# FFTAI/Wiki-GRx-Gym

Hardware: AMD Instinct MI355X
Metric: env-steps/sec GR1T1 rough-terrain @4096 envs (higher is better)
Workload: dtype f32

## Files before the change

wiki-grx-gym_amd/csrc/grx_step_kernel_body.inc:

```
    static_assert(!DBG || W == 1 || W == 4 || W == 8, "the debug injection path exists for the one-wave layout and the pipelines");
    KP P = GRX_PARAMS(Pg);
    constexpr int NTHR = 64 * W;
    constexpr bool PIPE = W >= 4;
    __shared__ KTables s_tab;
    constexpr int OBS_BYTES = EPB * GRX_NUM_OBS * 4, PRI_BYTES = EPB * PRS * 4, RW_BYTES = PIPE ? REWIN_FLOATS * 64 * 4 : 0;
    constexpr int POST_BYTES = OBS_BYTES + PRI_BYTES + RW_BYTES, PHYS_BYTES = (W == 2 || W == 8 ? 2 : 1) * RC_BYTES;
    static_assert(OBS_BYTES % 16 == 0 && PRI_BYTES % 16 == 0 && RC_BYTES % 16 == 0, "arena pieces must stay 16-byte aligned");
    constexpr int FOOTFR_BYTES = RC_FR4 * 64 * 16, ANCH_BYTES = 16 * 64 * 4;
    constexpr int TAIL_BYTES = PIPE ? PHYS_BYTES + FOOTFR_BYTES + ANCH_BYTES : PHYS_BYTES;
#ifdef GRX_FAKE_ARENA
    __shared__ __attribute__((aligned(16))) char s_arena[GRX_FAKE_ARENA];
#else
    __shared__ __attribute__((aligned(16))) char s_arena[POST_BYTES > TAIL_BYTES ? POST_BYTES : TAIL_BYTES];
#endif
    float* const s_obs = reinterpret_cast<float*>(s_arena);
    float* const s_pri = reinterpret_cast<float*>(s_arena + OBS_BYTES);
    float* const s_rw = reinterpret_cast<float*>(s_arena + OBS_BYTES + PRI_BYTES);
    static_assert(!PIPE || PHYS_BYTES >= OBS_BYTES + PRI_BYTES, "foot frames + s_anch must sit behind the staging rows, in the arena's tail");
    float4* const s_footfr = reinterpret_cast<float4*>(s_arena + PHYS_BYTES);
    float* const s_anch = reinterpret_cast<float*>(s_arena + PHYS_BYTES + FOOTFR_BYTES);
    __shared__ float s_stat[NSTAT];
    __shared__ float s_base[W == 2 ? 13 * EPB : 1];
    __shared__ float4 s_bq[PIPE ? 4 * EPB : 1];
    __shared__ __attribute__((aligned(16))) float s_wr[W == 2 ? 32 * 64 : (PIPE ? 8 * 64 : 1)];
    __shared__ float4 s_q[PIPE ? Q4 * 64 : 1];
    __shared__ float4 s_wc[PIPE ? WC4 * 64 : 1];
    __shared__ float4 s_pb[PIPE ? (LEG * PB4 + 2) * 64 : 1];
    __shared__ uint32_t s_nz[PIPE ? NZB * 4 * 64 : 1];
    __shared__ float4 s_rr[PIPE ? 5 * 64 : 1];
    __shared__ __attribute__((aligned(16))) char s_self[PIPE ? SELF_BYTES : 16];
    __shared__ float s_rwp[PIPE ? 64 : 1];
    __shared__ float s_hp[PIPE ? 4 * EPB : 1];
    __shared__ float s_hsum[PIPE ? W * 64 : 1];
    __shared__ float s_bho[W == 8 && HF ? 4 * 64 : 1];
    __shared__ float s_tp[PIPE ? 2 * 64 : 1];
    __shared__ float4 s_xk[W == 8 ? 9 * 64 : 1];
    __shared__ float4 s_sb[W == 8 ? 5 * 64 : 1];
    __shared__ float4 s_fx[W == 8 && LPL == 2 ? 8 * 64 : 1];
    __shared__ int s_flag[FL_COUNT];
    const PipeLds L = {s_bq, s_q, s_wc, s_pb, reinterpret_cast<float4*>(s_wr), s_flag, s_xk, s_sb, s_fx};
    const int tid = threadIdx.x;
#ifdef GRX_PROFILE_SECTIONS
    if (tid == 0) { P.prof[(size_t)blockIdx.x * GRX_PROF_SLOTS + 136] = (long long)__builtin_amdgcn_s_memrealtime(); P.prof[(size_t)blockIdx.x * GRX_PROF_SLOTS + 137] = clock64(); }
#endif
#ifndef GRX_W8_ROLES
#define GRX_W8_ROLES 0x76543210u
#endif
    const int wv_hw = __builtin_amdgcn_readfirstlane(tid >> 6);
    const int wv = W == 8 ? (int)((GRX_W8_ROLES >> (4 * wv_hw)) & 7u) : wv_hw;
    const RareBuf RB = rare_carve(s_arena + (W == 2 && wv == 1 ? RC_BYTES : 0));
    {
        const uint32_t* src = reinterpret_cast<const uint32_t*>(P.tables);
        uint32_t* dst = reinterpret_cast<uint32_t*>(&s_tab);
        for (int i = tid; i < (int)(sizeof(KTables) / 4); i += NTHR) dst[i] = src[i];
        if (tid < NSTAT) s_stat[tid] = 0.f;
        if (tid < FL_COUNT) s_flag[tid] = 0;
    }
    __syncthreads();
    if (wv == (W == 8 ? 3 : W - 1)) stats_fold_previous(P, sq, tid & 63);
    const int N = P.N;
    const int lane = tid & 63, el = lane_env(lane), side = lane_side(lane), half = lane_half(lane);
    const int grp = step_group();
    const int e_raw = grp * EPB + el;
    const bool act = e_raw < N;
    const bool act0 = act && half == 0;
    int e = act ? e_raw : N - 1;
    const SideConst& C = s_tab.side[side];
    const uint32_t genv = (uint32_t)(P.env_offset + e);
    const uint32_t step = (uint32_t)common_step;
    const int nh = P.nh, npri = P.num_pri_obs;
    const float dtp = P.sim_dt * (float)P.decimation;
    const int j0 = side * LEG;

#ifndef GRX_W8_PRIO
#define GRX_W8_PRIO 0u
#endif
    if (W == 8 && GRX_W8_PRIO) {
        const int pr = (int)((GRX_W8_PRIO >> (4 * wv)) & 3u);
        if (pr == 1) __builtin_amdgcn_s_setprio(1);
        else if (pr == 2) __builtin_amdgcn_s_setprio(2);
        else if (pr == 3) __builtin_amdgcn_s_setprio(3);
    }
    if (W >= 2 && wv != 0) {
        const float mu = 0.5f * (P.terrain_friction + P.friction[e]);
        float hmax = 0.0f;
        if (HF) {
            const float x0 = P.root[0 * (size_t)N + e], y0 = P.root[1 * (size_t)N + e];
            int ci = min(max((int)((x0 + P.border_size) / (P.horizontal_scale * (float)GRX_COARSE)), 0), P.coarse_rows - 1);
            int cj = min(max((int)((y0 + P.border_size) / (P.horizontal_scale * (float)GRX_COARSE)), 0), P.coarse_cols - 1);
            hmax = P.coarse_max[(size_t)ci * P.coarse_cols + cj];
        }
        LaneState hs;
        hs.anchor_on = 0;
        LinkPrep w3_lp;
        V3 w3_rows[11];
        if (PIPE) {
#if defined(GRX_REG_CONSTS) && GRX_REG_CONSTS >= 2
            const SideConst Ch = C;
#define GRX_HELPER_C Ch
#else
#define GRX_HELPER_C C
#endif
#ifndef GRX_W8_REGC
#define GRX_W8_REGC 0x76
#endif
#define GRX_HC(w) ((W == 8 && !((GRX_W8_REGC >> (w)) & 1)) ? C : GRX_HELPER_C)
            const float bm = P.base_m[e];
            const V3 bc = v3(P.base_c[e], P.base_c[(size_t)N + e], P.base_c[2 * (size_t)N + e]);
            const S3 bI = {P.base_I[e], P.base_I[(size_t)N + e], P.base_I[2 * (size_t)N + e],
                           P.base_I[3 * (size_t)N + e], P.base_I[4 * (size_t)N + e], P.base_I[5 * (size_t)N + e]};
            if (wv == 1) {
                const bool want_noise = P.add_noise && !noise_in;
                const int noise_seq = P.decimation >= 2 ? P.decimation - 2 : 0;
                auto noise_out = [&](const int seq) {
                    if (want_noise && seq == noise_seq) {
                        U4 nzb[NZB];
                        noise_blocks(P, genv, step, side, nzb);
                        uint32_t* z = s_nz + lane;
#pragma unroll
                        for (int b = 0; b < NZB; ++b) { z[(b * 4 + 0) * 64] = nzb[b].x; z[(b * 4 + 1) * 64] = nzb[b].y; z[(b * 4 + 2) * 64] = nzb[b].z; z[(b * 4 + 3) * 64] = nzb[b].w; }
                    }
                };
                if (DBG) noise_out(noise_seq);
                else self_loop<HF, HF && W != 8, W == 8>(P, s_tab, GRX_HC(1), RB, s_footfr, self_carve(s_self), P.friction[e], L, lane, el, side, noise_out);
            } else if (wv == 2) {
                constexpr int NA = 4 / LPL;
#pragma unroll
                for (int i = 0; i < NA; ++i) {
                    const int gi = NA * half + i;
                    hs.ax[i] = P.anchors[(size_t)((side * 4 + gi) * 3 + 0) * N + e];
                    hs.ay[i] = P.anchors[(size_t)((side * 4 + gi) * 3 + 1) * N + e];
                    hs.vimp[i] = P.anchors[(size_t)((side * 4 + gi) * 3 + 2) * N + e];
                    if (hs.vimp[i] != 0.0f) hs.anchor_on |= (1u << i);
                }
                V3 rpy_acc = v3(0.f, 0.f, 0.f);
                if (!DBG) chain_contact_loop<HF, W == 8 ? 0 : (HF ? 2 : 5)>(P, GRX_HC(2), C, RB, s_footfr, mu, hmax, 1.0f - 0.5f * (P.terrain_restitution + P.restitution[e]), hs, L, lane, el, side, rpy_acc);
                float* a_ = s_anch + (lane - half);
                if (half == 0) { a_[13 * 64] = rpy_acc.x; a_[14 * 64] = rpy_acc.y; a_[15 * 64] = rpy_acc.z; }
#pragma unroll
                for (int i = 0; i < NA; ++i) { const int gi = NA * half + i; a_[gi * 64] = hs.ax[i]; a_[(4 + gi) * 64] = hs.ay[i]; a_[(9 + gi) * 64] = hs.vimp[i]; }
                {
                    const uint32_t mine = hs.anchor_on << (NA * half);
                    a_[8 * 64] = __uint_as_float(LPL == 1 ? mine : (mine | __float_as_uint(half_swap(__uint_as_float(mine)))));
                }
            } else if (wv == 3) {
                if (DBG) { s_tp[lane] = dbg[(size_t)DBG_TERM_CONTACT * N + e]; s_tp[64 + lane] = 0.f; }
                else base_contact_loop<HF, W == 8>(P, s_tab, GRX_HC(3), RB, mu, hmax, bm, bc, bI, L, lane, el, side, s_tp, w3_lp, w3_rows, s_footfr, P.friction[e]);
            } else if (DBG) {
            } else if (wv == 7) {
                RareBuf RB7 = rare_carve(s_arena + RC_BYTES);
                RB7.fchain = RB.fchain;
                chain_rare_loop<HF>(P, s_tab, GRX_HC(7), RB7, mu, hmax, L, lane, el, side);
            } else if (wv == 4) {
                chain_bias_loop<3, 4>(P, GRX_HC(4), C, L, lane, el);
            } else if (wv == 6) {
                if (LPL == 1) chain_bias_loop<0, 2, true>(P, GRX_HC(6), C, L, lane, el, &s_tab, &RB, s_footfr, side, P.friction[e]);
                else chain_bias_loop<0, 2>(P, GRX_HC(6), C, L, lane, el);
            } else if (wv == 5) {
                base_service_loop(P, GRX_HC(5), C, bm, bc, bI, L, lane, el);
            }
            float es_w1[NT], es_w3[NT];
            if (wv == 1) load_episode_sums<1>(P, e, N, es_w1);
#ifdef GRX_PROFILE_SECTIONS
            if (lane == 0) P.prof[(size_t)blockIdx.x * GRX_PROF_SLOTS + 80 + wv] = clock64();
#endif
            lds_barrier();
            if (wv == 3) {
                load_episode_sums<2>(P, e, N, es_w3);
                if (!DBG) store_link_rows(LinkForceOut{true, act0 ? P.contact_forces + e : nullptr, (size_t)N}, w3_lp, w3_rows);
            }
            if (HF && P.measure_heights) {
                const float* hp = s_hp + el;
                if (W == 8) { if (wv != 3) { s_hsum[wv * 64 + lane] = height_scan_share<6, (LPE == 4 ? 6 : 11)>(P, s_tab, hp[2 * EPB], hp[3 * EPB], v3(hp[0 * EPB], hp[1 * EPB], 0.f),
                                                                                           LPE * (wv < 3 ? wv - 1 : wv - 2) + (lane & (LPE - 1)), nh, s_pri + el * PRS);
                                             flag_add(s_flag + FL_SCAN, lane); GRX_TICKV(96); } }
                else {
                s_hsum[wv * 64 + lane] = height_scan_share<4>(P, s_tab, hp[2 * EPB], hp[3 * EPB], v3(hp[0 * EPB], hp[1 * EPB], 0.f),
                                                              LPE * wv + (lane & (LPE - 1)), nh, s_pri + el * PRS);
                lds_barrier();
                }
            }
            if (wv == 2) {
                const ResetRand rr = reset_rand(P, genv, step, side);
                float4* z = s_rr + lane;
                z[0 * 64] = f4(rr.dof[0], rr.dof[1], rr.dof[2], rr.dof[3]);
                z[1 * 64] = f4(rr.dof[4], rr.root[0], rr.root[1], rr.root[2]);
                z[2 * 64] = f4(rr.root[3], rr.root[4], rr.root[5], rr.root[6]);
                z[3 * 64] = f4(rr.root[7], rr.root[8], rr.cmd[0], rr.cmd[1]);
                z[4 * 64] = f4(rr.cmd[2], 0.f, 0.f, 0.f);
                flag_set(s_flag + FL_RR, 1, lane);
                GRX_TICKV(104);
            }
            if (wv == 3) {
                flag_wait(s_flag + FL_REW, 1);
                RewIn rin;
                int i = 0;
                rewin_fields(rin, [&](float& x) { x = s_rw[(i++) * 64 + lane]; });
                if (W == 8 && HF) rin.feet_height = scan_feet_height(P, s_flag, s_hsum, rin.feet_height, nh, lane);
                reward_and_sums<2>(P, C, rin, lane, side, e, N, act, s_stat, es_w3, s_rwp, s_flag + FL_RWB, nullptr,
                                   DBG && dbg[(size_t)DBG_APPLY_RESET * N + e] == 0.f);
                GRX_TICKV(104);
            }
            if (wv == 1) {
                flag_wait(s_flag + FL_REW, 1);
                GRX_TICKW(14);
                RewIn rin;
                int i = 0;
                rewin_fields(rin, [&](float& x) { x = s_rw[(i++) * 64 + lane]; });
                if (W == 8 && HF) rin.feet_height = scan_feet_height(P, s_flag, s_hsum, rin.feet_height, nh, lane);
                float a_ll1[LEG];
                if (DBG) {
#pragma unroll
                    for (int k = 0; k < LEG; ++k) a_ll1[k] = dbg[(size_t)(DBG_LAST_LAST_ACTIONS + j0 + k) * N + e];
                }
                reward_and_sums<1>(P, C, rin, lane, side, e, N, act, s_stat, es_w1, s_rwp, s_flag + FL_RWB, DBG ? a_ll1 : nullptr,
                                   DBG && dbg[(size_t)DBG_APPLY_RESET * N + e] == 0.f);
                GRX_TICKW(15);
                GRX_TICKV(104);
            }
            if (W == 8) {
                if (wv >= 4) {
                    flag_wait(s_flag + FL_HZ, 1);
                    const bool have_raw = HF && P.measure_heights;
                    if (have_raw) flag_wait(s_flag + FL_SCAN, 6);
                    const float part = obs_heights_share<4 * LPE>(P, s_hp[el], (wv - 4) * LPE + (lane & (LPE - 1)), nh, s_pri + el * PRS, have_raw, act, e, N);
                    if (HF) s_bho[(wv - 4) * 64 + lane] = env_sum(part);
                    else s_hsum[wv * 64 + lane] = env_sum(part);
                    flag_set(s_flag + (wv == 7 ? FL_BHO4 : FL_BHO1 + (wv - 4)), 1, lane);
                    GRX_TICKV(112);
                }
            } else if (wv < 4) {
                flag_wait(s_flag + FL_HZ, 1);
                if (wv == 2) GRX_TICKW(30);
                const bool have_raw = HF && P.measure_heights;
                float* hrow = s_pri + el * PRS;
                const int li = lane & (LPE - 1);
                const float part = wv == 2 ? obs_heights_share<2 * LPE>(P, s_hp[el], li, nh, hrow, have_raw, act, e, N)
                                           : obs_heights_share<4 * LPE>(P, s_hp[el], (wv == 1 ? LPE : 3 * LPE) + li, nh, hrow, have_raw, act, e, N);
                s_hsum[wv * 64 + lane] = env_sum(part);
                flag_set(s_flag + FL_BHO1 + (wv - 1), 1, lane);
                if (wv == 2) GRX_TICKW(31);
            }
            if (P.publish_rbs && (W == 8 || wv < 4)) {
                float b_[13]; pipe_base_load(s_bq, el, b_);
                const float* b = b_;
                const float4 q0_ = s_q[lane], q1_ = s_q[64 + lane], q2_ = s_q[128 + lane];
                const float fq[LEG] = {q0_.x, q0_.y, q0_.z, q0_.w, q1_.x}, fqd[LEG] = {q1_.y, q1_.z, q1_.w, q2_.x, q2_.y};
                const float rq[4] = {b[3], b[4], b[5], b[6]};
                publish_rigid_body_states(P, C, side, v3(b[0], b[1], b[2]), rq, v3(b[7], b[8], b[9]),
                                          v3(b[10], b[11], b[12]), fq, fqd, e, N, act0, wv - 1, W == 8 ? 7 : 3);
            }
        } else {
            for (int deci = 0; deci < P.decimation; ++deci) {
                __syncthreads();
                const float* b = s_base + el;
                const V3 O = v3(b[0 * EPB], b[1 * EPB], b[2 * EPB]);
                const R3 R0 = quat_to_R(b[3 * EPB], b[4 * EPB], b[5 * EPB], b[6 * EPB]);
                const V3 vel = v3(b[7 * EPB], b[8 * EPB], b[9 * EPB]), ang = v3(b[10 * EPB], b[11 * EPB], b[12 * EPB]);
                RareOut ro;
                const ChainKin nok = {R0, v3(0.f, 0.f, 0.f), ang, vel};
                rare_contacts<HF, 0, 8>(P, s_tab, C, RB, lane, el, side, R0, O, ang, vel, nok, nok, mu, hmax, ro, nullptr, RareNoWait(), deci == P.decimation - 1);
                float* w_ = s_wr + lane;
                if (deci == P.decimation - 1) {
#pragma unroll
                    for (int i = 0; i < 8; ++i) { w_[(8 + 3 * i) * 64] = ro.lf[i].x; w_[(9 + 3 * i) * 64] = ro.lf[i].y; w_[(10 + 3 * i) * 64] = ro.lf[i].z; }
                }
                w_[0 * 64] = ro.f0a.x; w_[1 * 64] = ro.f0a.y; w_[2 * 64] = ro.f0a.z;
                w_[3 * 64] = ro.f0l.x; w_[4 * 64] = ro.f0l.y; w_[5 * 64] = ro.f0l.z;
                w_[6 * 64] = ro.term ? 1.f : 0.f; w_[7 * 64] = ro.pen_count;
                __syncthreads();
            }
        }
    } else {

#ifdef GRX_PROFILE_SECTIONS
    long long tacc[22] = {};
#else
    long long* tacc = nullptr;
#endif
    GRX_TICK(0);
    LaneState st;
    LaneConst LC;
    float a_cur[LEG], a_last[LEG], qd_last[LEG];
#pragma unroll
    for (int k = 0; k < LEG; ++k) {
        size_t o = (size_t)(j0 + k) * N + e;
        st.q[k] = GCOL(P.q, o); st.qd[k] = GCOL(P.qd, o);
        a_last[k] = GCOL(P.last_actions, o);
        LC.strength[k] = GCOL(P.motor_strength, o);
        float a = actions_in ? actions_in[(size_t)e * GRX_ND + j0 + k] : 0.0f;
        a_cur[k] = fminf(fmaxf(a, C.body[k].amin), C.body[k].amax);
    }
    st.pos = v3(GCOL(P.root, 0 * (size_t)N + e), GCOL(P.root, 1 * (size_t)N + e), GCOL(P.root, 2 * (size_t)N + e));
    st.qx = GCOL(P.root, 3 * (size_t)N + e); st.qy = GCOL(P.root, 4 * (size_t)N + e); st.qz = GCOL(P.root, 5 * (size_t)N + e); st.qw = GCOL(P.root, 6 * (size_t)N + e);
    st.vel = v3(GCOL(P.root, 7 * (size_t)N + e), GCOL(P.root, 8 * (size_t)N + e), GCOL(P.root, 9 * (size_t)N + e));
    st.ang = v3(GCOL(P.root, 10 * (size_t)N + e), GCOL(P.root, 11 * (size_t)N + e), GCOL(P.root, 12 * (size_t)N + e));
#pragma unroll
    for (int i = 0; i < 4; ++i) {
        st.ax[i] = GCOL(P.anchors, (size_t)((side * 4 + i) * 3 + 0) * N + e);
        st.ay[i] = GCOL(P.anchors, (size_t)((side * 4 + i) * 3 + 1) * N + e);
    }
    st.anchor_on = 0;
#pragma unroll
    for (int i = 0; i < 4; ++i) {
        st.vimp[i] = GCOL(P.anchors, (size_t)((side * 4 + i) * 3 + 2) * N + e);
        if (st.vimp[i] != 0.0f) st.anchor_on |= (1u << i);
    }
    LC.base_m = GCOL(P.base_m, e);
    LC.base_c = v3(GCOL(P.base_c, e), GCOL(P.base_c, (size_t)N + e), GCOL(P.base_c, 2 * (size_t)N + e));
    LC.base_I.xx = P.base_I[e]; LC.base_I.xy = P.base_I[(size_t)N + e]; LC.base_I.xz = P.base_I[2 * (size_t)N + e];
    LC.base_I.yy = P.base_I[3 * (size_t)N + e]; LC.base_I.yz = P.base_I[4 * (size_t)N + e]; LC.base_I.zz = P.base_I[5 * (size_t)N + e];
    LC.mu = 0.5f * (P.terrain_friction + GCOL(P.friction, e));
    LC.om_e = 1.0f - 0.5f * (P.terrain_restitution + GCOL(P.restitution, e));
    LC.hmax = 0.0f;
    if (HF) {
        int ci = min(max((int)((st.pos.x + P.border_size) / (P.horizontal_scale * (float)GRX_COARSE)), 0), P.coarse_rows - 1);
        int cj = min(max((int)((st.pos.y + P.border_size) / (P.horizontal_scale * (float)GRX_COARSE)), 0), P.coarse_cols - 1);
        LC.hmax = P.coarse_max[(size_t)ci * P.coarse_cols + cj];
    }
    EnvAux ea;
    float air_time, land_time, bho_stale;
    bool contact_last;
    long long ep_len;
    auto load_post_state = [&]() {
#pragma unroll
// ... 138 lines not shown
        GCOL(P.avg_speed_rpy, (size_t)(side * 3 + 0) * N + e) = (avg_rpy.x + fabsf(fk.ang.x)) * id;
        GCOL(P.avg_speed_rpy, (size_t)(side * 3 + 1) * N + e) = (avg_rpy.y + fabsf(fk.ang.y)) * id;
        GCOL(P.avg_speed_rpy, (size_t)(side * 3 + 2) * N + e) = (avg_rpy.z + fabsf(fk.ang.z)) * id;
    }
    float a_ll[LEG];
    bool dbg_apply_reset = true;
    if (DBG) {
        const float* d = dbg + e;
        const size_t n_ = (size_t)N;
        so.foot_force = v3(d[(DBG_FEET_FORCE + side * 3 + 0) * n_], d[(DBG_FEET_FORCE + side * 3 + 1) * n_], d[(DBG_FEET_FORCE + side * 3 + 2) * n_]);
        fk.pos = v3(d[(DBG_FEET_POS + side * 3 + 0) * n_], d[(DBG_FEET_POS + side * 3 + 1) * n_], d[(DBG_FEET_POS + side * 3 + 2) * n_]);
        avg_force = d[(DBG_AVG_FORCE + side) * n_];
        avg_speed = v3(d[(DBG_AVG_SPEED + side * 3 + 0) * n_], d[(DBG_AVG_SPEED + side * 3 + 1) * n_], d[(DBG_AVG_SPEED + side * 3 + 2) * n_]);
#pragma unroll
        for (int k = 0; k < LEG; ++k) { torque[k] = d[(DBG_TORQUES + j0 + k) * n_]; a_ll[k] = d[(DBG_LAST_LAST_ACTIONS + j0 + k) * n_]; }
        if (!PIPE) { so.term = d[DBG_TERM_CONTACT * n_] != 0.f; so.pen_count = 0.f; }
        dbg_apply_reset = d[DBG_APPLY_RESET * n_] != 0.f;
    }
    const bool term_contact = __builtin_bit_cast(int, pair_swap(__builtin_bit_cast(float, (int)so.term))) | (int)so.term;
    const float pen_count = pair_sum(so.pen_count);

    GRX_TICK(3);
    float es_early[NT];
    if (!PIPE) {
#pragma unroll
        for (int t = 0; t < NT; ++t) es_early[t] = (P.reward_scale_dt[t] != 0.f) ? GCOL(P.episode_sums, (size_t)t * N + e) : 0.f;
    }
    ep_len += 1;
    V3 qv = v3(st.qx, st.qy, st.qz);
    V3 blv = quat_rotate_inverse(qv, st.qw, st.vel);
    V3 bav = quat_rotate_inverse(qv, st.qw, st.ang);
    V3 pg = quat_rotate_inverse(qv, st.qw, v3(0.f, 0.f, -1.f));
    if (P.resample_command_interval > 0 && ((uint32_t)ep_len % (uint32_t)P.resample_command_interval) == 0)
        resample_commands(P, genv, step, GRX_RNG_CMD_TIME, ea.cmd);
    if (!PIPE && P.heading_command) ea.cmd[2] = heading_yaw_command(P, v3(st.qx, st.qy, st.qz), st.qw);
    float* prow = s_pri + el * PRS;
    float hsum = 0.f;
    if (HF && P.measure_heights) {
        if (PIPE) {
            if (W != 8) {
            hsum = height_scan_share<4>(P, s_tab, yaw_z, yaw_w, st.pos, lane & (LPE - 1), nh, prow);
            lds_barrier();
            hsum += s_hsum[1 * 64 + lane] + s_hsum[2 * 64 + lane] + s_hsum[3 * 64 + lane];
            }
        } else hsum = height_scan_share<1, GRX_W1_SCAN_BATCH>(P, s_tab, yaw_z, yaw_w, st.pos, lane & (LPE - 1), nh, prow);
        hsum = env_sum(hsum);
    }
    if (P.push_robots && P.push_interval > 0 && (step % (uint32_t)P.push_interval) == 0) {
        if (P.stash_pre_reset && act0 && side == 0) { P.pre_push_vel[e] = st.vel.x; P.pre_push_vel[(size_t)N + e] = st.vel.y; }
        st.vel.x = urand(P, genv, step, GRX_RNG_PUSH, 0, -P.max_push_vel_xy, P.max_push_vel_xy);
        st.vel.y = urand(P, genv, step, GRX_RNG_PUSH, 1, -P.max_push_vel_xy, P.max_push_vel_xy);
    }
    GRX_TICK(4);
    const bool contact = so.foot_force.z > 1.0f;
    const bool contact_filt = contact || contact_last;
    contact_last = contact;
    const bool first_contact = (air_time > 0.f) && contact_filt;
    air_time += dtp;
    constexpr bool kLateScan = PIPE && W == 8 && HF;
    const bool late_scan = kLateScan && P.measure_heights;
    float feet_height = late_scan ? fk.pos.z : (nh > 0 ? (fk.pos.z * (float)nh - hsum) / (float)nh : fk.pos.z);
    land_time = (land_time + dtp) * (contact ? 1.0f : 0.0f);
    bool reset = term_contact || (fabsf(pg.z) < P.termination_gravity_z);
    const bool time_out = (float)ep_len > P.max_episode_length;
    reset = reset || time_out;

    GRX_TICK(5);
    {
        RewIn rin;
#pragma unroll
        for (int k = 0; k < LEG; ++k) {
            rin.a_last[k] = a_last[k]; rin.a_cur[k] = a_cur[k]; rin.q[k] = st.q[k]; rin.qd[k] = st.qd[k];
            rin.qd_last[k] = qd_last[k]; rin.torque[k] = torque[k];
        }
        rin.feet_height = feet_height; rin.air_time = air_time; rin.land_time = land_time; rin.avg_force = avg_force;
        rin.avg_speed = avg_speed; rin.foot_force = so.foot_force;
        rin.contact = contact ? 1.f : 0.f; rin.first_contact = first_contact ? 1.f : 0.f;
        rin.cmd[0] = ea.cmd[0]; rin.cmd[1] = ea.cmd[1]; rin.cmd[2] = ea.cmd[2];
        rin.blv = blv; rin.bav = bav; rin.pg = pg;
        rin.bho_stale = bho_stale; rin.qx = st.qx; rin.qy = st.qy; rin.qz = st.qz; rin.qw = st.qw; rin.pen_count = pen_count;
        rin.reset = reset ? 1.f : 0.f; rin.time_out = time_out ? 1.f : 0.f;
        if (PIPE) {
            int i = 0;
            rewin_fields(rin, [&](float& x) { s_rw[(i++) * 64 + lane] = x; });
            flag_set(s_flag + FL_REW, 1, lane);
        } else if constexpr (kBaseTerms) {
            const float base_z = nh > 0 ? st.pos.z - hsum / (float)nh : st.pos.z;
            const float rb = base_reward_and_sums(P, C, rin, base_z, lane, side, e, N, act, grp, DBG && !dbg_apply_reset);
            reward_and_sums<0, true>(P, C, rin, lane, side, e, N, act, s_stat, es_early, nullptr, nullptr, DBG ? a_ll : nullptr, DBG && !dbg_apply_reset, rb);
        } else reward_and_sums<0>(P, C, rin, lane, side, e, N, act, s_stat, es_early, nullptr, nullptr, DBG ? a_ll : nullptr, DBG && !dbg_apply_reset);
    }
    const bool writer = act0 && side == 0;
    GRX_TICK(6);
    const bool do_reset = DBG ? (reset && dbg_apply_reset) : reset;
    if (P.stash_pre_reset && reset && act0) {
        const size_t n_ = (size_t)N;
#pragma unroll
        for (int k = 0; k < LEG; ++k) { P.pre_q[(size_t)(side * LEG + k) * n_ + e] = st.q[k]; P.pre_qd[(size_t)(side * LEG + k) * n_ + e] = st.qd[k]; }
        if (side == 0) {
            float* r_ = P.pre_root + e;
            r_[0] = st.pos.x; r_[n_] = st.pos.y; r_[2 * n_] = st.pos.z; r_[3 * n_] = st.qx; r_[4 * n_] = st.qy; r_[5 * n_] = st.qz; r_[6 * n_] = st.qw;
            r_[7 * n_] = st.vel.x; r_[8 * n_] = st.vel.y; r_[9 * n_] = st.vel.z; r_[10 * n_] = st.ang.x; r_[11 * n_] = st.ang.y; r_[12 * n_] = st.ang.z;
        }
    }
    if (PIPE ? __any(do_reset) : do_reset) {
        ResetRand rr;
        if (PIPE) {
            flag_wait(s_flag + FL_RR, 1);
            const float4* z = s_rr + lane;
            const float4 z0 = z[0 * 64], z1 = z[1 * 64], z2 = z[2 * 64], z3 = z[3 * 64], z4 = z[4 * 64];
            rr.dof[0] = z0.x; rr.dof[1] = z0.y; rr.dof[2] = z0.z; rr.dof[3] = z0.w; rr.dof[4] = z1.x;
            rr.root[0] = z1.y; rr.root[1] = z1.z; rr.root[2] = z1.w; rr.root[3] = z2.x; rr.root[4] = z2.y;
            rr.root[5] = z2.z; rr.root[6] = z2.w; rr.root[7] = z3.x; rr.root[8] = z3.y;
            rr.cmd[0] = z3.z; rr.cmd[1] = z3.w; rr.cmd[2] = z4.x;
        } else rr = reset_rand(P, genv, step, side);
      if (do_reset) {
        reset_env(P, C, side, genv, step, true, st, ea, rr);
#pragma unroll
        for (int k = 0; k < LEG; ++k) { a_last[k] = 0.f; qd_last[k] = 0.f; }
        air_time = 0.f; land_time = 0.f;
        contact_last = false;
        ep_len = 0;
      }
    }
    const bool feet_contact_obs = do_reset ? false : contact;
    {
        const float ls = level_sum(ea.level, writer);
        if (lane == 0) s_stat[NT + 1] = ls;
    }

    GRX_TICK(7);
    float bho = 0.f;
    if (PIPE) {
        if (side == 0) s_hp[el] = st.pos.z;
        flag_set(s_flag + FL_HZ, 1, lane);
    } else {
        const float sum = env_sum(obs_heights_share<LPE>(P, st.pos.z, lane & (LPE - 1), nh, prow, HF && P.measure_heights, act, e, N));
        bho = nh > 0 ? sum / (float)nh : 0.f;
    }
    GRX_TICK(11);
    float* orow = s_obs + el * GRX_NUM_OBS;
    const float clipo = P.clip_observations;
    U4 nzb[NZB];
    if (P.add_noise && !noise_in) {
        if (PIPE) {
            const uint32_t* z = s_nz + lane;
#pragma unroll
            for (int b = 0; b < NZB; ++b) { nzb[b].x = z[(b * 4 + 0) * 64]; nzb[b].y = z[(b * 4 + 1) * 64]; nzb[b].z = z[(b * 4 + 2) * 64]; nzb[b].w = z[(b * 4 + 3) * 64]; }
        } else noise_blocks(P, genv, step, side, nzb);
    }
    GRX_TICK(12);
    auto put = [&](int idx, float val, float nscale, int item, int slot0) {
        float pv = fminf(fmaxf(val, -clipo), clipo);
        prow[idx] = pv;
        float ov = val;
        if (P.add_noise && nscale != 0.f) {
            float u;
            if (noise_in) u = noise_in[(size_t)e * GRX_NUM_OBS + idx];
            else {
                const U4 o = nzb[slot0 + (item >> 2)];
                const int wsel = item & 3;
                u = grx_u01(wsel == 0 ? o.x : (wsel == 1 ? o.y : (wsel == 2 ? o.z : o.w)));
            }
            ov += (2.f * u - 1.f) * nscale;
        }
        orow[idx] = fminf(fmaxf(ov, -clipo), clipo);
    };
    if (side == 0) {
        put(0, ea.cmd[0], 0.f, 0, 4); put(1, ea.cmd[1], 0.f, 0, 4); put(2, ea.cmd[2], 0.f, 0, 4);
        const float na = P.noise_ang_vel * P.noise_level * P.obs_scale_ang_vel;
        put(3, bav.x * P.obs_scale_ang_vel, na, 0, 4); put(4, bav.y * P.obs_scale_ang_vel, na, 1, 4); put(5, bav.z * P.obs_scale_ang_vel, na, 2, 4);
        const float ng = P.noise_gravity * P.noise_level * P.obs_scale_gravity;
        put(6, pg.x * P.obs_scale_gravity, ng, 3, 4); put(7, pg.y * P.obs_scale_gravity, ng, 4, 4); put(8, pg.z * P.obs_scale_gravity, ng, 5, 4);
        prow[GRX_NUM_OBS + 0] = fminf(fmaxf(blv.x * P.obs_scale_lin_vel, -clipo), clipo);
        prow[GRX_NUM_OBS + 1] = fminf(fmaxf(blv.y * P.obs_scale_lin_vel, -clipo), clipo);
        prow[GRX_NUM_OBS + 2] = fminf(fmaxf(blv.z * P.obs_scale_lin_vel, -clipo), clipo);
    }
    GRX_TICK(13);
    {
        const float np_ = P.noise_dof_pos * P.noise_level * P.obs_scale_dof_pos;
        const float nv = P.noise_dof_vel * P.noise_level * P.obs_scale_dof_vel;
        const float nac = P.noise_action * P.noise_level * P.obs_scale_action;
#pragma unroll
        for (int k = 0; k < LEG; ++k) {
            put(9 + j0 + k, (st.q[k] - C.body[k].q0) * P.obs_scale_dof_pos, np_, k, 0);
            put(9 + GRX_ND + j0 + k, st.qd[k] * P.obs_scale_dof_vel, nv, 5 + k, 0);
            put(9 + 2 * GRX_ND + j0 + k, a_cur[k] * P.obs_scale_action, nac, 10 + k, 0);
        }
        if (late_scan) feet_height = scan_feet_height(P, s_flag, s_hsum, feet_height, nh, lane);
        prow[GRX_NUM_OBS + 4 + side] = feet_contact_obs ? 1.f : 0.f;
        prow[GRX_NUM_OBS + 6 + side] = fminf(fmaxf(feet_height * P.obs_scale_height, -clipo), clipo);
    }
    if (!PIPE && side == 0) prow[GRX_NUM_OBS + 3] = fminf(fmaxf(bho * P.obs_scale_height, -clipo), clipo);

    GRX_TICK(8);
    if (act0) {
#pragma unroll
        for (int k = 0; k < LEG; ++k) {
            size_t o = (size_t)(j0 + k) * N + e;
            GCOL(P.q, o) = st.q[k]; GCOL(P.qd, o) = st.qd[k];
            GCOL(P.last_actions, o) = a_cur[k]; GCOL(P.last_dof_vel, o) = st.qd[k];
            GCOL(P.actions, o) = a_cur[k]; GCOL(P.torques, o) = torque[k];
        }
#pragma unroll
        for (int i = 0; i < 4; ++i) {
            GCOL(P.anchors, (size_t)((side * 4 + i) * 3 + 0) * N + e) = st.ax[i];
            GCOL(P.anchors, (size_t)((side * 4 + i) * 3 + 1) * N + e) = st.ay[i];
            GCOL(P.anchors, (size_t)((side * 4 + i) * 3 + 2) * N + e) = (st.anchor_on >> i) & 1u ? fmaxf(st.vimp[i], 1e-6f) : 0.f;
        }
        GCOL(P.air_time, (size_t)side * N + e) = air_time * (contact_filt ? 0.f : 1.f);
        GCOL(P.land_time, (size_t)side * N + e) = land_time;
        GCOL(P.feet_contact, (size_t)side * N + e) = feet_contact_obs ? 1 : 0;
        GCOL(P.feet_height, (size_t)side * N + e) = feet_height;
        GCOL(P.avg_force, (size_t)side * N + e) = avg_force;
#pragma unroll
        for (int i = 0; i < 3; ++i) {
            float ff = i == 0 ? so.foot_force.x : (i == 1 ? so.foot_force.y : so.foot_force.z);
            float fp = i == 0 ? fk.pos.x : (i == 1 ? fk.pos.y : fk.pos.z);
            float as_ = i == 0 ? avg_speed.x : (i == 1 ? avg_speed.y : avg_speed.z);
            GCOL(P.feet_force, (size_t)(side * 3 + i) * N + e) = ff;
            GCOL(P.feet_pos, (size_t)(side * 3 + i) * N + e) = fp;
            GCOL(P.avg_speed, (size_t)(side * 3 + i) * N + e) = as_;
        }
    }
    GRX_TICK(93);
    if (writer) {
        float rs[13] = {st.pos.x, st.pos.y, st.pos.z, st.qx, st.qy, st.qz, st.qw, st.vel.x, st.vel.y, st.vel.z, st.ang.x, st.ang.y, st.ang.z};
#pragma unroll
        for (int i = 0; i < 13; ++i) GCOL(P.root, (size_t)i * N + e) = rs[i];
        GCOL(P.commands, e) = ea.cmd[0]; GCOL(P.commands, (size_t)N + e) = ea.cmd[1]; GCOL(P.commands, 2 * (size_t)N + e) = ea.cmd[2];
        GCOL(P.base_lin_vel, e) = blv.x; GCOL(P.base_lin_vel, (size_t)N + e) = blv.y; GCOL(P.base_lin_vel, 2 * (size_t)N + e) = blv.z;
        GCOL(P.base_ang_vel, e) = bav.x; GCOL(P.base_ang_vel, (size_t)N + e) = bav.y; GCOL(P.base_ang_vel, 2 * (size_t)N + e) = bav.z;
        GCOL(P.proj_grav, e) = pg.x; GCOL(P.proj_grav, (size_t)N + e) = pg.y; GCOL(P.proj_grav, 2 * (size_t)N + e) = pg.z;
        GCOL(P.origins, e) = ea.origin[0]; GCOL(P.origins, (size_t)N + e) = ea.origin[1]; GCOL(P.origins, 2 * (size_t)N + e) = ea.origin[2];
        GCOL(P.levels, e) = ea.level;
        if (!PIPE) GCOL(P.base_heights_offset, e) = bho;
        GCOL(P.ep_len, e) = ep_len;
        GCOL(P.reset, e) = reset ? 1 : 0;
        GCOL(P.time_out, e) = time_out ? 1 : 0;
        GCOL(P.term_contact, e) = term_contact ? 1 : 0;
    }
    GRX_TICK(94);
    if (PIPE) {
        if (W == 8) {
            flag_wait_all(s_flag, flag_want(lane, FL_BHO1, 1, FL_BHO1 + 1, 1, FL_BHO1 + 2, 1, FL_BHO4, 1), lane);
            if (HF) bho = nh > 0 ? ((s_bho[0 * 64 + lane] + s_bho[1 * 64 + lane]) + (s_bho[2 * 64 + lane] + s_bho[3 * 64 + lane])) / (float)nh : 0.f;
            else bho = nh > 0 ? ((s_hsum[4 * 64 + lane] + s_hsum[5 * 64 + lane]) + (s_hsum[6 * 64 + lane] + s_hsum[7 * 64 + lane])) / (float)nh : 0.f;
        } else {
        flag_wait(s_flag + FL_BHO1, 1);
        flag_wait(s_flag + FL_BHO1 + 1, 1);
        flag_wait(s_flag + FL_BHO1 + 2, 1);
        bho = nh > 0 ? (s_hsum[1 * 64 + lane] + s_hsum[2 * 64 + lane] + s_hsum[3 * 64 + lane]) / (float)nh : 0.f;
        }
        if (side == 0) prow[GRX_NUM_OBS + 3] = fminf(fmaxf(bho * P.obs_scale_height, -clipo), clipo);
        if (writer) GCOL(P.base_heights_offset, e) = bho;
    }
    GRX_TICK(9);
    }
    GRX_TICKV(120);
    lds_barrier();
    {
        const int e0 = grp * EPB;
        const int nenv = min(EPB, N - e0);
        float* gobs = (obs_out ? obs_out : P.obs) + (size_t)e0 * GRX_NUM_OBS;
        const int tot = nenv * GRX_NUM_OBS;
        if (nenv == EPB) {
            const float4* s4 = reinterpret_cast<const float4*>(s_obs);
            float4* g4 = reinterpret_cast<float4*>(gobs);
            for (int i = tid; i < EPB * GRX_NUM_OBS / 4; i += NTHR) g4[i] = s4[i];
        } else
            for (int i = tid; i < tot; i += NTHR) gobs[i] = s_obs[i];
        float* gpri = (pri_out ? pri_out : P.pri_obs) + (size_t)e0 * npri;
        if (npri == GRX_MAX_PRI && nenv == EPB) {
            const float2* s2 = reinterpret_cast<const float2*>(s_pri);
            float2* g2 = reinterpret_cast<float2*>(gpri);
            for (int i = tid; i < EPB * GRX_MAX_PRI / 2; i += NTHR) {
                const int row = i / (GRX_MAX_PRI / 2);
                g2[i] = s2[i + row * ((PRS - GRX_MAX_PRI) / 2)];
            }
        } else
            for (int i = tid; i < nenv * npri; i += NTHR) gpri[i] = s_pri[(i / npri) * PRS + (i % npri)];
        if (tid < NSTAT) stat_row(P, sq.seq, tid)[grp] = s_stat[tid];
        if (blockIdx.x == 0 && tid == 0) P.stat_nblocks[sq.seq & 1] = (int)gridDim.x;
    }
    GRX_TICK(10);
    GRX_TICKV(128);
#ifdef GRX_PROFILE_SECTIONS
    if ((tid & 63) == 0) P.prof[(size_t)blockIdx.x * GRX_PROF_SLOTS + 144 + wv] = (long long)__builtin_amdgcn_s_memrealtime();
#endif
```

wiki-grx-gym_amd/csrc/grx_wavepipe.h:

```cpp
#pragma once
#ifndef GRX_W8_WAITALL
#define GRX_W8_WAITALL 1
#endif
#ifndef GRX_W8_RARESPLIT
#define GRX_W8_RARESPLIT 1
#endif

#ifdef GRX_PROFILE_SECTIONS
#define GRX_HELPER_PROF_BEGIN long long hp_idle = 0, hp_t0 = clock64(), hp_t = 0
#define GRX_HELPER_PROF_IDLE0 hp_t = clock64()
#define GRX_HELPER_PROF_IDLE1 hp_idle += clock64() - hp_t
#define GRX_HELPER_PROF_END(w) do { if (lane == 0) { P.prof[(size_t)blockIdx.x * GRX_PROF_SLOTS + 22 + 2 * (w)] = hp_idle; P.prof[(size_t)blockIdx.x * GRX_PROF_SLOTS + 23 + 2 * (w)] = clock64() - hp_t0; } } while (0)
#else
#define GRX_HELPER_PROF_BEGIN do {} while (0)
#define GRX_HELPER_PROF_IDLE0 do {} while (0)
#define GRX_HELPER_PROF_IDLE1 do {} while (0)
#define GRX_HELPER_PROF_END(w) do {} while (0)
#endif

#ifdef GRX_PROFILE_SECTIONS
#define GRX_EV(i) do { if ((seq == 5 || seq == 0) && lane == 0) { __builtin_amdgcn_sched_barrier(0); P.prof[(size_t)blockIdx.x * GRX_PROF_SLOTS + (seq == 5 ? 48 : 160) + (i)] = clock64(); __builtin_amdgcn_sched_barrier(0); } } while (0)
#else
#define GRX_EV(i) do {} while (0)
#endif
#define GRX_PIN(x) asm volatile("" : "+v"(x))
#ifdef GRX_PROFILE_SECTIONS
#define GRX_WAIT(f, want, slot) do { long long w0_ = clock64(); flag_wait(f, want); tacc[slot] += clock64() - w0_; } while (0)
#define GRX_WAIT_ALL(f, want_mine, lane, slot) do { long long w0_ = clock64(); flag_wait_all(f, want_mine, lane); tacc[slot] += clock64() - w0_; } while (0)
#else
#define GRX_WAIT(f, want, slot) flag_wait(f, want)
#define GRX_WAIT_ALL(f, want_mine, lane, slot) flag_wait_all(f, want_mine, lane)
#endif

enum { FL_STATE = 0, FL_FOOT = 2, FL_LEGS = 3, FL_FRAMES = 4, FL_BIAS = 5, FL_BIAS2 = 7 , FL_SELF = 9, FL_REW = 6, FL_BASEBIAS = 8, FL_HZ = 10, FL_BHO1 = 11 , FL_RWB = 14, FL_RR = 15,
       FL_FACT = 16 , FL_FACTOUT = 17 ,
       FL_XK = 18 ,
       FL_CHAINW = 19 , FL_BHO4 = 20 ,
       FL_SB = 21 ,
       FL_SCAN = 1 ,
       FL_COUNT = 22 };
constexpr bool flag_slots_distinct() {
    const int f[] = {FL_STATE, FL_SCAN, FL_FOOT, FL_LEGS, FL_FRAMES, FL_BIAS, FL_REW, FL_BIAS2, FL_BASEBIAS, FL_SELF, FL_HZ, FL_BHO1, FL_BHO1 + 1, FL_BHO1 + 2, FL_RWB, FL_RR,
                     FL_FACT, FL_FACTOUT, FL_XK, FL_CHAINW, FL_BHO4, FL_SB};
    constexpr int n = sizeof(f) / sizeof(f[0]);
    for (int i = 0; i < n; ++i) {
        if (f[i] < 0 || f[i] >= FL_COUNT) return false;
        for (int j = i + 1; j < n; ++j) if (f[i] == f[j]) return false;
    }
    return n == FL_COUNT;
}
static_assert(flag_slots_distinct(), "hand-over flags must occupy distinct slots of s_flag, all of them");
constexpr int PB4 = 2;
constexpr int WC4 = 15;
constexpr int Q4 = 3;

struct PipeLds {
    float4* bq;
    float4* q;
    float4* wc;
    float4* pb;
    float4* wr;
    int* flag;
    float4* xk;
    float4* sb;
    float4* fx;
};
GRX_DEV float4 f4(float a, float b, float c, float d) { float4 r; r.x = a; r.y = b; r.z = c; r.w = d; return r; }
GRX_DEV void pipe_base_load(const float4* bq, int el, float b[13]) {
    const float4 a = bq[el], c = bq[EPB + el], d = bq[2 * EPB + el], e = bq[3 * EPB + el];
    b[0] = a.x; b[1] = a.y; b[2] = a.z; b[3] = a.w; b[4] = c.x; b[5] = c.y; b[6] = c.z; b[7] = c.w;
    b[8] = d.x; b[9] = d.y; b[10] = d.z; b[11] = d.w; b[12] = e.x;
}
GRX_DEV void pipe_base_store(float4* bq, int el, V3 pos, float qx, float qy, float qz, float qw, V3 vel, V3 ang) {
    bq[el] = f4(pos.x, pos.y, pos.z, qx); bq[EPB + el] = f4(qy, qz, qw, vel.x);
    bq[2 * EPB + el] = f4(vel.y, vel.z, ang.x, ang.y); bq[3 * EPB + el] = f4(ang.z, 0.f, 0.f, 0.f);
}

#include "grx_flags.h"

GRX_DEV void rigid_bias(const R3& R, V3 kap, float m, const S3& Ic, V3 w, V3 v, V3& pa, V3& pl) {
    const V3 l = (v + cross(w, kap)) * m;
    const V3 Lc = rot(R, mul(Ic, rotT(R, w)));
    const V3 ha = Lc + cross(kap, l);
    pa = cross(w, ha) + cross(v, l);
    pl = cross(w, l);
}

GRX_DEV void rigid_inertia(const R3& R, V3 kap, float m, const S3& Ic, S3& A, V3& h) {
    A = rot_sym(R, Ic);
    const float kk = dot(kap, kap);
    A.xx += m * (kk - kap.x * kap.x); A.xy -= m * kap.x * kap.y; A.xz -= m * kap.x * kap.z;
    A.yy += m * (kk - kap.y * kap.y); A.yz -= m * kap.y * kap.z; A.zz += m * (kk - kap.z * kap.z);
    h = kap * m;
}
GRX_DEV void add_rigid(S3& A, M3& B, S3& D, const S3& Ak, V3 h, float m) {
    A = A + Ak;
    B.a01 -= h.z; B.a02 += h.y; B.a10 += h.z; B.a12 -= h.x; B.a20 -= h.y; B.a21 += h.x;
    D.xx += m; D.yy += m; D.zz += m;
}

template <int HF, bool W8>
GRX_DEV void substep_p(KP P, const SideConst& C, const LaneConst& LC, LaneState& st, const float tau_m[LEG],
                       SubstepOut& out, FootKin& fk_before, const PipeLds& L, const RareBuf& RB, int lane, int seq, long long* tacc,
                       const SideConst& Clds) {
    const float dt = P.sim_dt;
#ifdef GRX_PROFILE_SECTIONS
    long long tprev = clock64();
#endif
    V3 Sa[LEG], Ss[LEG], ca[LEG], cl[LEG], Ua[LEG], Ul[LEG];
    float dinv[LEG], uu[LEG];
    GRX_EV(0);
    S3 AK[LEG];
    V3 hK[LEG];
    const R3 R0 = quat_to_R(st.qx, st.qy, st.qz, st.qw);
    {
        R3 R = R0;
        V3 rho = v3(0.f, 0.f, 0.f), w = st.ang, v = st.vel;
#pragma unroll
        for (int k = 0; k < LEG; ++k) {
            const float qdk = st.qd[k];
            rho = rho + rot(R, v3(C.body[k].r[0], C.body[k].r[1], C.body[k].r[2]));
            float sn, cs;
            grx_sincos(st.q[k], sn, cs);
            R = joint_rot_k(R, cs, sn, kAxis[k]);
            const V3 a = axis_k(R, kAxis[k]);
            const V3 s_ = cross(rho, a);
            Sa[k] = a; Ss[k] = s_;
            if (!W8) {
                ca[k] = cross(w, a) * qdk;
                cl[k] = (cross(v, a) + cross(w, s_)) * qdk;
                w = fma3(a, qdk, w); v = fma3(s_, qdk, v);
            }
#ifndef GRX_P8_XK
#define GRX_P8_XK 1
#endif
            if (W8 && GRX_P8_XK && k < 2) continue;
            const V3 kap = rho + rot(R, v3(C.body[k].com[0], C.body[k].com[1], C.body[k].com[2]));
// ... 1047 lines not shown
```

Measured before the change: 96.74 million.

## Split post-reset tail work across helper waves via an LDS record

In the 8-wave pipeline layout, the main wave no longer builds observations and writes every state column to global memory after the reset. It packs the post-reset per-leg and per-env state into an LDS record and raises flags. Wave 2 then builds the noisy, clipped observation rows, and waves 4-7 split the global state stores between them. Reward inputs are also staged as float4 rows instead of scalar rows. The aim is to take the tail off the critical wave and overlap it, at the cost of extra LDS traffic, flag synchronisation and arena space.

New measurement: 98.09 million, median of 6. +1.4%, better.

```diff
diff --git a/wiki-grx-gym_amd/csrc/grx_step_kernel_body.inc b/wiki-grx-gym_amd/csrc/grx_step_kernel_body.inc
--- a/wiki-grx-gym_amd/csrc/grx_step_kernel_body.inc
+++ b/wiki-grx-gym_amd/csrc/grx_step_kernel_body.inc
@@ -3,7 +3,12 @@
     constexpr int NTHR = 64 * W;
     constexpr bool PIPE = W >= 4;
     __shared__ KTables s_tab;
-    constexpr int OBS_BYTES = EPB * GRX_NUM_OBS * 4, PRI_BYTES = EPB * PRS * 4, RW_BYTES = PIPE ? REWIN_FLOATS * 64 * 4 : 0;
+#ifndef GRX_TAIL_SPLIT
+#define GRX_TAIL_SPLIT 1
+#endif
+    constexpr bool kTailSplit = GRX_TAIL_SPLIT && PIPE && W == 8 && LPL == 2;
+    constexpr int REWIN4 = (REWIN_FLOATS + 3) / 4;
+    constexpr int OBS_BYTES = EPB * GRX_NUM_OBS * 4, PRI_BYTES = EPB * PRS * 4, RW_BYTES = PIPE ? (kTailSplit ? REWIN4 * 64 * 16 : REWIN_FLOATS * 64 * 4) : 0;
     constexpr int POST_BYTES = OBS_BYTES + PRI_BYTES + RW_BYTES, PHYS_BYTES = (W == 2 || W == 8 ? 2 : 1) * RC_BYTES;
     static_assert(OBS_BYTES % 16 == 0 && PRI_BYTES % 16 == 0 && RC_BYTES % 16 == 0, "arena pieces must stay 16-byte aligned");
     constexpr int FOOTFR_BYTES = RC_FR4 * 64 * 16, ANCH_BYTES = 16 * 64 * 4;
@@ -39,6 +44,10 @@
     __shared__ float4 s_fx[W == 8 && LPL == 2 ? 8 * 64 : 1];
     __shared__ int s_flag[FL_COUNT];
     const PipeLds L = {s_bq, s_q, s_wc, s_pb, reinterpret_cast<float4*>(s_wr), s_flag, s_xk, s_sb, s_fx};
+    constexpr int REC_OFF = (POST_BYTES + 15) / 16 * 16;
+    static_assert(!kTailSplit || REC_OFF + (TAIL_LEG4 + TAIL_ENV4) * 64 * 16 <= PHYS_BYTES + FOOTFR_BYTES, "the post-reset record must fit between the reward inputs and s_anch");
+    float4* const s_rec = reinterpret_cast<float4*>(s_arena + (kTailSplit ? REC_OFF : 0));
+    float4* const s_renv = s_rec + TAIL_LEG4 * 64;
     const int tid = threadIdx.x;
 #ifdef GRX_PROFILE_SECTIONS
     if (tid == 0) { P.prof[(size_t)blockIdx.x * GRX_PROF_SLOTS + 136] = (long long)__builtin_amdgcn_s_memrealtime(); P.prof[(size_t)blockIdx.x * GRX_PROF_SLOTS + 137] = clock64(); }
@@ -195,6 +204,13 @@
                 flag_wait(s_flag + FL_REW, 1);
                 RewIn rin;
                 int i = 0;
+                if (kTailSplit) {
+                    float w_[4 * REWIN4];
+                    const float4* z = reinterpret_cast<const float4*>(s_rw) + lane;
+#pragma unroll
+                    for (int r = 0; r < REWIN4; ++r) { const float4 t = z[r * 64]; w_[4 * r] = t.x; w_[4 * r + 1] = t.y; w_[4 * r + 2] = t.z; w_[4 * r + 3] = t.w; }
+                    rewin_fields(rin, [&](float& x) { x = w_[i++]; });
+                } else
                 rewin_fields(rin, [&](float& x) { x = s_rw[(i++) * 64 + lane]; });
                 if (W == 8 && HF) rin.feet_height = scan_feet_height(P, s_flag, s_hsum, rin.feet_height, nh, lane);
                 reward_and_sums<2>(P, C, rin, lane, side, e, N, act, s_stat, es_w3, s_rwp, s_flag + FL_RWB, nullptr,
@@ -206,6 +222,13 @@
                 GRX_TICKW(14);
                 RewIn rin;
                 int i = 0;
+                if (kTailSplit) {
+                    float w_[4 * REWIN4];
+                    const float4* z = reinterpret_cast<const float4*>(s_rw) + lane;
+#pragma unroll
+                    for (int r = 0; r < REWIN4; ++r) { const float4 t = z[r * 64]; w_[4 * r] = t.x; w_[4 * r + 1] = t.y; w_[4 * r + 2] = t.z; w_[4 * r + 3] = t.w; }
+                    rewin_fields(rin, [&](float& x) { x = w_[i++]; });
+                } else
                 rewin_fields(rin, [&](float& x) { x = s_rw[(i++) * 64 + lane]; });
                 if (W == 8 && HF) rin.feet_height = scan_feet_height(P, s_flag, s_hsum, rin.feet_height, nh, lane);
                 float a_ll1[LEG];
@@ -241,6 +264,130 @@
                 flag_set(s_flag + FL_BHO1 + (wv - 1), 1, lane);
                 if (wv == 2) GRX_TICKW(31);
             }
+            if (kTailSplit && wv == 2) {
+                U4 nzb[NZB];
+                if (P.add_noise && !noise_in) {
+                    const uint32_t* z = s_nz + lane;
+#pragma unroll
+                    for (int b = 0; b < NZB; ++b) { nzb[b].x = z[(b * 4 + 0) * 64]; nzb[b].y = z[(b * 4 + 1) * 64]; nzb[b].z = z[(b * 4 + 2) * 64]; nzb[b].w = z[(b * 4 + 3) * 64]; }
+                }
+                flag_wait(s_flag + FL_HZ, 2);
+                const float4* r_ = s_rec + lane;
+                const float4 r0 = r_[0 * 64], r1 = r_[1 * 64], r2 = r_[2 * 64], r3 = r_[3 * 64], r8 = r_[8 * 64], r11 = r_[11 * 64];
+                const float oq[LEG] = {r0.x, r0.y, r0.z, r0.w, r1.x}, oqd[LEG] = {r1.y, r1.z, r1.w, r2.x, r2.y}, oa[LEG] = {r2.z, r2.w, r3.x, r3.y, r3.z};
+                float* prow = s_pri + el * PRS;
+                float* orow = s_obs + el * GRX_NUM_OBS;
+                const float clipo = P.clip_observations;
+                auto put = [&](int idx, float val, float nscale, int item, int slot0) {
+                    float pv = fminf(fmaxf(val, -clipo), clipo);
+                    prow[idx] = pv;
+                    float ov = val;
+                    if (P.add_noise && nscale != 0.f) {
+                        float u;
+                        if (noise_in) u = noise_in[(size_t)e * GRX_NUM_OBS + idx];
+                        else {
+                            const U4 o = nzb[slot0 + (item >> 2)];
+                            const int wsel = item & 3;
+                            u = grx_u01(wsel == 0 ? o.x : (wsel == 1 ? o.y : (wsel == 2 ? o.z : o.w)));
+                        }
+                        ov += (2.f * u - 1.f) * nscale;
+                    }
+                    orow[idx] = fminf(fmaxf(ov, -clipo), clipo);
+                };
+                if (side == 0) {
+                    const float4* v_ = s_renv + lane;
+                    const float4 v3_ = v_[3 * 64], v4 = v_[4 * 64], v5 = v_[5 * 64], v6 = v_[6 * 64];
+                    const V3 blv = v3(v4.x, v4.y, v4.z), bav = v3(v4.w, v5.x, v5.y), pg = v3(v5.z, v5.w, v6.x);
+                    put(0, v3_.y, 0.f, 0, 4); put(1, v3_.z, 0.f, 0, 4); put(2, v3_.w, 0.f, 0, 4);
+                    const float na = P.noise_ang_vel * P.noise_level * P.obs_scale_ang_vel;
+                    put(3, bav.x * P.obs_scale_ang_vel, na, 0, 4); put(4, bav.y * P.obs_scale_ang_vel, na, 1, 4); put(5, bav.z * P.obs_scale_ang_vel, na, 2, 4);
+                    const float ng = P.noise_gravity * P.noise_level * P.obs_scale_gravity;
+                    put(6, pg.x * P.obs_scale_gravity, ng, 3, 4); put(7, pg.y * P.obs_scale_gravity, ng, 4, 4); put(8, pg.z * P.obs_scale_gravity, ng, 5, 4);
+                    prow[GRX_NUM_OBS + 0] = fminf(fmaxf(blv.x * P.obs_scale_lin_vel, -clipo), clipo);
+                    prow[GRX_NUM_OBS + 1] = fminf(fmaxf(blv.y * P.obs_scale_lin_vel, -clipo), clipo);
+                    prow[GRX_NUM_OBS + 2] = fminf(fmaxf(blv.z * P.obs_scale_lin_vel, -clipo), clipo);
+                }
+                const float np_ = P.noise_dof_pos * P.noise_level * P.obs_scale_dof_pos;
+                const float nv = P.noise_dof_vel * P.noise_level * P.obs_scale_dof_vel;
+                const float nac = P.noise_action * P.noise_level * P.obs_scale_action;
+#pragma unroll
+                for (int k = 0; k < LEG; ++k) {
+                    put(9 + j0 + k, (oq[k] - C.body[k].q0) * P.obs_scale_dof_pos, np_, k, 0);
+                    put(9 + GRX_ND + j0 + k, oqd[k] * P.obs_scale_dof_vel, nv, 5 + k, 0);
+                    put(9 + 2 * GRX_ND + j0 + k, oa[k] * P.obs_scale_action, nac, 10 + k, 0);
+                }
+                float feet_height = r11.y;
+                if (HF && P.measure_heights) feet_height = scan_feet_height(P, s_flag, s_hsum, feet_height, nh, lane);
+                prow[GRX_NUM_OBS + 4 + side] = r8.z;
+                prow[GRX_NUM_OBS + 6 + side] = fminf(fmaxf(feet_height * P.obs_scale_height, -clipo), clipo);
+                if (act0) GCOL(P.feet_height, (size_t)side * N + e) = feet_height;
+                GRX_TICKV(152);
+            } else if (kTailSplit && wv >= 4) {
+                flag_wait(s_flag + FL_HZ, 3);
+                const float4* r_ = s_rec + lane;
+                if (wv == 4) {
+                    if (act0 && side == 0) {
+                        const float4* v_ = s_renv + lane;
+                        const float4 v0 = v_[0 * 64], v1 = v_[1 * 64], v2 = v_[2 * 64], v3_ = v_[3 * 64], v4 = v_[4 * 64], v5 = v_[5 * 64], v6 = v_[6 * 64], v7 = v_[7 * 64], v8 = v_[8 * 64];
+                        const float rs[13] = {v0.x, v0.y, v0.z, v0.w, v1.x, v1.y, v1.z, v1.w, v2.x, v2.y, v2.z, v2.w, v3_.x};
+#pragma unroll
+                        for (int i = 0; i < 13; ++i) GCOL(P.root, (size_t)i * N + e) = rs[i];
+                        GCOL(P.commands, e) = v3_.y; GCOL(P.commands, (size_t)N + e) = v3_.z; GCOL(P.commands, 2 * (size_t)N + e) = v3_.w;
+                        GCOL(P.base_lin_vel, e) = v4.x; GCOL(P.base_lin_vel, (size_t)N + e) = v4.y; GCOL(P.base_lin_vel, 2 * (size_t)N + e) = v4.z;
+                        GCOL(P.base_ang_vel, e) = v4.w; GCOL(P.base_ang_vel, (size_t)N + e) = v5.x; GCOL(P.base_ang_vel, 2 * (size_t)N + e) = v5.y;
+                        GCOL(P.proj_grav, e) = v5.z; GCOL(P.proj_grav, (size_t)N + e) = v5.w; GCOL(P.proj_grav, 2 * (size_t)N + e) = v6.x;
+                        GCOL(P.origins, e) = v6.y; GCOL(P.origins, (size_t)N + e) = v6.z; GCOL(P.origins, 2 * (size_t)N + e) = v6.w;
+                        GCOL(P.levels, e) = __float_as_int(v7.x);
+                        GCOL(P.ep_len, e) = (long long)(((unsigned long long)__float_as_uint(v7.z) << 32) | (unsigned long long)__float_as_uint(v7.y));
+                        GCOL(P.reset, e) = __float_as_int(v7.w);
+                        GCOL(P.time_out, e) = __float_as_int(v8.x);
+                        GCOL(P.term_contact, e) = __float_as_int(v8.y);
+                    }
+                } else if (wv == 5) {
+                    const float4 r0 = r_[0 * 64], r1 = r_[1 * 64], r2 = r_[2 * 64], r8 = r_[8 * 64];
+                    const float oq[LEG] = {r0.x, r0.y, r0.z, r0.w, r1.x}, oqd[LEG] = {r1.y, r1.z, r1.w, r2.x, r2.y};
+                    if (act0) {
+#pragma unroll
+                        for (int k = 0; k < LEG; ++k) {
+                            const size_t o = (size_t)(j0 + k) * N + e;
+                            GCOL(P.q, o) = oq[k]; GCOL(P.qd, o) = oqd[k]; GCOL(P.last_dof_vel, o) = oqd[k];
+                        }
+                        GCOL(P.air_time, (size_t)side * N + e) = r8.x;
+                        GCOL(P.land_time, (size_t)side * N + e) = r8.y;
+                        GCOL(P.feet_contact, (size_t)side * N + e) = r8.z != 0.f ? 1 : 0;
+                        GCOL(P.avg_force, (size_t)side * N + e) = r8.w;
+                    }
+                } else if (wv == 6) {
+                    const float4 r5 = r_[5 * 64], r6 = r_[6 * 64], r7 = r_[7 * 64], r9 = r_[9 * 64], r10 = r_[10 * 64], r11 = r_[11 * 64];
+                    const float ax[4] = {r5.x, r5.y, r5.z, r5.w}, ay[4] = {r6.x, r6.y, r6.z, r6.w}, av[4] = {r7.x, r7.y, r7.z, r7.w};
+                    const float ff[3] = {r9.x, r9.y, r9.z}, fp[3] = {r9.w, r10.x, r10.y}, as_[3] = {r10.z, r10.w, r11.x};
+                    if (act0) {
+#pragma unroll
+                        for (int i = 0; i < 4; ++i) {
+                            GCOL(P.anchors, (size_t)((side * 4 + i) * 3 + 0) * N + e) = ax[i];
+                            GCOL(P.anchors, (size_t)((side * 4 + i) * 3 + 1) * N + e) = ay[i];
+                            GCOL(P.anchors, (size_t)((side * 4 + i) * 3 + 2) * N + e) = av[i];
+                        }
+#pragma unroll
+                        for (int i = 0; i < 3; ++i) {
+                            GCOL(P.feet_force, (size_t)(side * 3 + i) * N + e) = ff[i];
+                            GCOL(P.feet_pos, (size_t)(side * 3 + i) * N + e) = fp[i];
+                            GCOL(P.avg_speed, (size_t)(side * 3 + i) * N + e) = as_[i];
+                        }
+                    }
+                } else {
+                    const float4 r2 = r_[2 * 64], r3 = r_[3 * 64], r4 = r_[4 * 64];
+                    const float oa[LEG] = {r2.z, r2.w, r3.x, r3.y, r3.z}, ot[LEG] = {r3.w, r4.x, r4.y, r4.z, r4.w};
+                    if (act0) {
+#pragma unroll
+                        for (int k = 0; k < LEG; ++k) {
+                            const size_t o = (size_t)(j0 + k) * N + e;
+                            GCOL(P.last_actions, o) = oa[k]; GCOL(P.actions, o) = oa[k]; GCOL(P.torques, o) = ot[k];
+                        }
+                    }
+                }
+                GRX_TICKV(152);
+            }
             if (P.publish_rbs && (W == 8 || wv < 4)) {
                 float b_[13]; pipe_base_load(s_bq, el, b_);
                 const float* b = b_;
@@ -545,6 +692,13 @@
         rin.reset = reset ? 1.f : 0.f; rin.time_out = time_out ? 1.f : 0.f;
         if (PIPE) {
             int i = 0;
+            if (kTailSplit) {
+                float w_[4 * REWIN4] = {};
+                rewin_fields(rin, [&](float& x) { w_[i++] = x; });
+                float4* z = reinterpret_cast<float4*>(s_rw) + lane;
+#pragma unroll
+                for (int r = 0; r < REWIN4; ++r) z[r * 64] = f4(w_[4 * r], w_[4 * r + 1], w_[4 * r + 2], w_[4 * r + 3]);
+            } else
             rewin_fields(rin, [&](float& x) { s_rw[(i++) * 64 + lane] = x; });
             flag_set(s_flag + FL_REW, 1, lane);
         } else if constexpr (kBaseTerms) {
@@ -602,8 +756,40 @@
         bho = nh > 0 ? sum / (float)nh : 0.f;
     }
     GRX_TICK(11);
+    const float clipo = P.clip_observations;
+    if (kTailSplit) {
+        float4* r_ = s_rec + lane;
+        float4* v_ = s_renv + lane;
+        r_[0 * 64] = f4(st.q[0], st.q[1], st.q[2], st.q[3]);
+        r_[1 * 64] = f4(st.q[4], st.qd[0], st.qd[1], st.qd[2]);
+        r_[2 * 64] = f4(st.qd[3], st.qd[4], a_cur[0], a_cur[1]);
+        r_[3 * 64] = f4(a_cur[2], a_cur[3], a_cur[4], torque[0]);
+        r_[8 * 64] = f4(air_time * (contact_filt ? 0.f : 1.f), land_time, feet_contact_obs ? 1.f : 0.f, avg_force);
+        r_[11 * 64] = f4(avg_speed.z, feet_height, 0.f, 0.f);
+        v_[3 * 64] = f4(st.ang.z, ea.cmd[0], ea.cmd[1], ea.cmd[2]);
+        v_[4 * 64] = f4(blv.x, blv.y, blv.z, bav.x);
+        v_[5 * 64] = f4(bav.y, bav.z, pg.x, pg.y);
+        v_[6 * 64] = f4(pg.z, ea.origin[0], ea.origin[1], ea.origin[2]);
+        flag_set(s_flag + FL_HZ, 2, lane);
+        r_[4 * 64] = f4(torque[1], torque[2], torque[3], torque[4]);
+        r_[5 * 64] = f4(st.ax[0], st.ax[1], st.ax[2], st.ax[3]);
+        r_[6 * 64] = f4(st.ay[0], st.ay[1], st.ay[2], st.ay[3]);
+        float av[4];
+#pragma unroll
+        for (int i = 0; i < 4; ++i) av[i] = (st.anchor_on >> i) & 1u ? fmaxf(st.vimp[i], 1e-6f) : 0.f;
+        r_[7 * 64] = f4(av[0], av[1], av[2], av[3]);
+        r_[9 * 64] = f4(so.foot_force.x, so.foot_force.y, so.foot_force.z, fk.pos.x);
+        r_[10 * 64] = f4(fk.pos.y, fk.pos.z, avg_speed.x, avg_speed.y);
+        v_[0 * 64] = f4(st.pos.x, st.pos.y, st.pos.z, st.qx);
+        v_[1 * 64] = f4(st.qy, st.qz, st.qw, st.vel.x);
+        v_[2 * 64] = f4(st.vel.y, st.vel.z, st.ang.x, st.ang.y);
+        v_[7 * 64] = f4(__int_as_float(ea.level), __int_as_float((int)(uint32_t)(unsigned long long)ep_len), __int_as_float((int)(uint32_t)((unsigned long long)ep_len >> 32)),
+                        __int_as_float(reset ? 1 : 0));
+        v_[8 * 64] = f4(__int_as_float(time_out ? 1 : 0), __int_as_float(term_contact ? 1 : 0), 0.f, 0.f);
+        flag_set(s_flag + FL_HZ, 3, lane);
+        GRX_TICK(8);
+    } else {
     float* orow = s_obs + el * GRX_NUM_OBS;
-    const float clipo = P.clip_observations;
     U4 nzb[NZB];
     if (P.add_noise && !noise_in) {
         if (PIPE) {
@@ -702,6 +888,7 @@
         GCOL(P.reset, e) = reset ? 1 : 0;
         GCOL(P.time_out, e) = time_out ? 1 : 0;
         GCOL(P.term_contact, e) = term_contact ? 1 : 0;
+    }
     }
     GRX_TICK(94);
     if (PIPE) {
diff --git a/wiki-grx-gym_amd/csrc/grx_wavepipe.h b/wiki-grx-gym_amd/csrc/grx_wavepipe.h
--- a/wiki-grx-gym_amd/csrc/grx_wavepipe.h
+++ b/wiki-grx-gym_amd/csrc/grx_wavepipe.h
@@ -53,6 +53,7 @@
 constexpr int PB4 = 2;
 constexpr int WC4 = 15;
 constexpr int Q4 = 3;
+constexpr int TAIL_LEG4 = 12, TAIL_ENV4 = 9;
 
 struct PipeLds {
     float4* bq;
```
